# Blaizzy/mlx-audio-swift

Hardware: AMD Instinct MI355X
Metric: audio-seconds/sec (TTS gen+codec decode), Orpheus-3B batch 32 per GPU: value = whole-job aggregate over n_gpus, value_per_gpu = value / n_gpus (higher is better)
Workload: dtype bf16

## Files before the change

### include/mi_speech_debug.h

```cpp
#ifndef MI_SPEECH_DEBUG_H
#define MI_SPEECH_DEBUG_H
#include "mi_speech.h"
#ifdef __cplusplus
extern "C" {
#endif

mis_status mis_debug_launch_floor(int device, int n_kernels, int mode, int reps, double* us_per_kernel);
int32_t mis_debug_choose_split(int32_t items, int32_t k_tiles, int32_t waves_per_item, int32_t s_max);
mis_status mis_debug_occupy_cus(int device, int blocks, int threads, double seconds);
mis_status mis_debug_occupy_wait(void);
int32_t mis_debug_device_cus(int device);
int32_t mis_debug_sampler_failures(void);
int64_t mis_debug_whisper_weight_bytes(const mis_whisper* c);
mis_status mis_debug_mimi_decoder_tap(mis_mimi* m, const int32_t* codes, int batch, int n_q, int T, int stage, float* out, int64_t capacity,
                                      int32_t* channels, int64_t* length);

mis_status mis_debug_gemm_skinny(int device, const uint16_t* W, const uint16_t* W2, const uint16_t* X, const uint16_t* bias, int M, int N, int K,
                                 int epi, int R, int ksb, int U, int S, float* out, int64_t capacity, int32_t* report);
mis_status mis_debug_gemm_skinny_q(int device, int bits, int sb_dtype, const uint32_t* wq, const uint16_t* scales, const uint16_t* biases,
                                   const uint32_t* wq2, const uint16_t* scales2, const uint16_t* biases2, const uint16_t* X, const uint16_t* bias,
                                   int M, int N, int K, int epi, int R, int ksb, int S, float* out, int64_t capacity, int32_t* report);
mis_status mis_debug_gemm_pf(int device, const uint16_t* W, const uint16_t* W2, const uint16_t* X, const uint16_t* h, int M, int N, int K, int epi,
                             float* out, int64_t capacity, int32_t* report);

typedef struct mis_debug_attn_args {
    int32_t batch, Mpad, S, Nqkv, H, Hkv, D, Smax;
    int32_t cache_rows, append_only, first_schedule, cross, cross_len, out_ld, rope_in_dtype;
    int32_t qp_S, qp_KT;
    float scale, qk_eps, qp_eps;
    const float* qkv_part;
    const int32_t* pos;
    const uint8_t* active;
    const float *rope_cos, *rope_sin;
    const uint16_t *qnorm_w, *knorm_w;
    const uint16_t* qp_w;
// ... 92 lines not shown
```

### mlx-audio-swift_amd/_lib.py

```python
from __future__ import annotations

import ctypes as C
import os

_HERE = os.path.dirname(os.path.abspath(__file__))
LIB_PATH = os.environ.get("MIS_LIB_PATH") or os.path.join(_HERE, "libmi_speech.so")

MIS_OK = 0
STATUS_NAMES = {0: "ok", 1: "modelNotInitialized", 2: "generationFailed", 3: "invalidInput",
                4: "audioDecodingFailed", 5: "audioEncodingFailed", 6: "cancelled", 7: "device"}
MIS_F32, MIS_F16, MIS_BF16, MIS_I32 = 0, 1, 2, 3
EVENT_TOKEN, EVENT_INFO, EVENT_AUDIO = 0, 1, 2


class SnacConfigC(C.Structure):
    _fields_ = [("sampling_rate", C.c_int32), ("latent_dim", C.c_int32), ("decoder_dim", C.c_int32),
                ("n_decoder_rates", C.c_int32), ("decoder_rates", C.c_int32 * 8), ("codebook_size", C.c_int32),
                ("codebook_dim", C.c_int32), ("n_codebooks", C.c_int32), ("vq_strides", C.c_int32 * 8),
                ("noise", C.c_int32), ("depthwise", C.c_int32), ("attn_window_size", C.c_int32)]


class LmConfigC(C.Structure):
    _fields_ = [("hidden_size", C.c_int32), ("num_hidden_layers", C.c_int32), ("intermediate_size", C.c_int32),
                ("num_attention_heads", C.c_int32), ("num_key_value_heads", C.c_int32), ("head_dim", C.c_int32),
# ... 391 lines not shown
}

class AttnDebugArgsC(C.Structure):
    _fields_ = ([(n, C.c_int32) for n in ("batch", "Mpad", "S", "Nqkv", "H", "Hkv", "D", "Smax", "cache_rows", "append_only", "first_schedule",
                                          "cross", "cross_len", "out_ld", "rope_in_dtype", "qp_S", "qp_KT")] +
                [(n, C.c_float) for n in ("scale", "qk_eps", "qp_eps")] +
                [(n, _P) for n in ("qkv_part", "pos", "active", "rope_cos", "rope_sin", "qnorm_w", "knorm_w", "qp_w", "qp_bias", "qp_slabs",
                                   "qp_h_in", "qp_lnw", "qp_lnb", "kcache", "vtcache", "kcache_out", "vtcache_out", "out", "qp_h_out", "report")])


class CodecGemmDebugArgsC(C.Structure):
    _fields_ = ([(n, C.c_int32) for n in ("mode", "snake", "batch", "use_pack", "M", "K", "N", "Tin", "Tout", "s", "pad", "Cin", "ldx", "ldy",
                                          "x_lo", "dup_bias_n0", "split_k_ok", "taps", "dil", "noise_rng")] +
                [("noise_key", C.c_uint64), ("row_offset", C.c_int64)] +
                [(n, _P) for n in ("AT", "bias", "X", "R", "scale", "noise", "alpha", "ralpha", "row_ids", "Y", "report")])


DEBUG_SYMBOLS = {
    "mis_debug_launch_floor": (C.c_int, [C.c_int, C.c_int, C.c_int, C.c_int, C.POINTER(C.c_double)]),
    "mis_debug_occupy_cus": (C.c_int, [C.c_int, C.c_int, C.c_int, C.c_double]),
    "mis_debug_occupy_wait": (C.c_int, []),
    "mis_debug_device_cus": (C.c_int32, [C.c_int]),
    "mis_debug_sampler_failures": (C.c_int32, []),
    "mis_debug_choose_split": (C.c_int32, [C.c_int32, C.c_int32, C.c_int32, C.c_int32]),
    "mis_debug_gemm_skinny": (C.c_int, [C.c_int, _P, _P, _P, _P, C.c_int, C.c_int, C.c_int, C.c_int, C.c_int, C.c_int, C.c_int, C.c_int, _P,
                                        C.c_int64, _P]),
    "mis_debug_gemm_skinny_q": (C.c_int, [C.c_int, C.c_int, C.c_int, _P, _P, _P, _P, _P, _P, _P, _P, C.c_int, C.c_int, C.c_int, C.c_int, C.c_int,
                                          C.c_int, C.c_int, _P, C.c_int64, _P]),
    "mis_debug_gemm_pf": (C.c_int, [C.c_int, _P, _P, _P, _P, C.c_int, C.c_int, C.c_int, C.c_int, _P, C.c_int64, _P]),
    "mis_debug_attn_decode": (C.c_int, [C.c_int, C.POINTER(AttnDebugArgsC)]),
    "mis_debug_codec_gemm": (C.c_int, [C.c_int, C.POINTER(CodecGemmDebugArgsC)]),
    "mis_debug_codec_final": (C.c_int, [C.c_int, _P, _P, C.c_float, _P, _P, C.c_int, C.c_int, C.c_int, C.c_int, C.c_int, C.c_int, C.c_int64, _P]),
    "mis_debug_codec_hist": (C.c_int, [C.c_int, _P, _P, C.c_int, C.c_int, C.c_int, C.c_int, C.c_int, _P, _P]),
    "mis_debug_codec_embed": (C.c_int, [C.c_int, _P, C.c_int64, C.c_int64, C.c_int64, C.c_int64, _P, C.c_int, C.c_int, C.c_int, C.c_int, C.c_int,
                                        C.c_int, _P]),
    "mis_debug_codec_dw7": (C.c_int, [C.c_int, _P, _P, _P, C.c_int, C.c_int, C.c_int, C.c_int, _P]),
    "mis_debug_codec_vq_nearest": (C.c_int, [C.c_int, _P, _P, _P, C.c_int, C.c_int, C.c_int, C.c_int, _P]),
    "mis_debug_gemm_big": (C.c_int, [C.c_int, C.c_int, _P, _P, _P, _P, C.c_int, C.c_int, C.c_int, C.c_int, C.c_int, _P, _P]),
    "mis_debug_enc_layernorm": (C.c_int, [C.c_int, _P, _P, _P, C.c_int, C.c_int, C.c_float, _P, _P]),
    "mis_debug_enc_im2col3": (C.c_int, [C.c_int, _P, C.c_int, C.c_int, C.c_int, C.c_int, C.c_int, C.c_int, _P]),
    "mis_debug_enc_scatter_kv": (C.c_int, [C.c_int, _P, C.c_int, C.c_int, C.c_int, C.c_int, C.c_int, C.c_int, C.c_int, C.c_int, _P, _P]),
    "mis_debug_enc_attn_prefill": (C.c_int, [C.c_int, _P, C.c_int, _P, _P, C.c_int, C.c_int, C.c_int, C.c_int, C.c_int, C.c_int, _P, _P]),
    "mis_debug_whisper_embed_ln": (C.c_int, [C.c_int, _P, _P, _P, _P, _P, _P, _P, _P, C.c_int, C.c_int, C.c_int, C.c_int, C.c_int, _P, _P]),
    "mis_debug_whisper_suppress": (C.c_int, [C.c_int, _P, C.c_int, C.c_int, _P, C.c_int, _P, C.c_int, _P, _P, C.c_int]),
    "mis_debug_lm_embed_rmsnorm": (C.c_int, [C.c_int, _P, _P, _P, _P, _P, _P, C.c_int, C.c_int, C.c_float, C.c_int, C.c_int, _P, _P]),
    "mis_debug_lm_glue": (C.c_int, [C.c_int, _P, C.c_int, C.c_int, C.c_int, _P, _P, _P, C.c_float, _P, _P]),
# ... 55 lines not shown
```

### mlx-audio-swift_amd/csrc/lm_engine.hip

```cpp
#include <deque>
#include <map>
#include "common.h"
#include "kernels.h"
#include "lm_kernels.h"

#include <math.h>
#include <string.h>
#include <algorithm>
#include <chrono>
#include <functional>
#include <set>

#define ORPHEUS_END_OF_SPEECH 128258

struct mis_tts {
    int device = 0;
    hipStream_t stream = nullptr;
    mis_lm_config cfg{};
    mis_snac* codec = nullptr;
    int d = 0, L = 0, ff = 0, H = 0, Hkv = 0, D = 0, V = 0, Vpad = 0, Nqkv = 0;
    bool finalized = false, have_lm_head = false;
    std::set<std::string> loaded;

    DevBuf<bf16_t> emb;
// ... 16 lines not shown
    } q_qkv, q_o, q_gu, q_down, q_head;

    int batch = 0, Mpad = 0, Smax = 0;
    int S_qkv = 1, S_o = 1, S_down = 1;
    int r_part = 1;
    int r_gu = 2;
    int ksb_part = 4, ksb_gu = 4, ksb_head = 1;
    GemmArr a_qkv, a_o, a_down, a_head;
    GemmArr qa_gu, qa_head;
    DevBuf<bf16_t> kcache, vtcache;
    DevBuf<float> rope_cos, rope_sin;
    DevBuf<int32_t> ids, pos_cur, pos_next;
    DevBuf<uint8_t> active;
    DevBuf<bf16_t> h, x, attn_out, act, logits;
    DevBuf<float> qkv_part, part, e_buf, logits_f32, samp_l32;
    DevBuf<int32_t> prompt_mat, prompt_lens, step_counter, window, window_len, n_gen, tokens_out, all_ids, all_len,
        done_count, codes, n_codes, l0, l1, l2, row_map;
    DevBuf<float> pcm_tmp;
    DevBuf<bf16_t> pf_h, pf_x, pf_attn, pf_act, pf_xpk, pf_actpk;
    DevBuf<float> pf_qkv, pf_tmp;
    DevBuf<int32_t> pf_pos;
    DevBuf<uint8_t> pf_on;
    DevBuf<SamplerScratch> samp_scratch;
    hipGraphExec_t g_prefill = nullptr, g_decode = nullptr;
    bool shared_device = false;
    uint64_t graph_key = 0;
    bool use_graph = true;
    bool borrowed_stream = false;
    bool rope_csm = false;
    int profiling = 0;
    mis_tts_timing timing{};
    SamplerParams sp{};
};

static size_t layer_qkv_elems(const mis_tts* c) { return (size_t)c->Nqkv * c->d; }
static size_t layer_o_elems(const mis_tts* c) { return (size_t)c->d * c->H * c->D; }
static size_t layer_gu_elems(const mis_tts* c) { return (size_t)2 * c->ff * c->d; }
static size_t layer_down_elems(const mis_tts* c) { return (size_t)c->d * c->ff; }

extern "C" mis_status mis_tts_create(const mis_lm_config* cfg, mis_snac* codec, int device, mis_tts** out) {
    MIS_API_BEGIN
    MIS_REQUIRE(cfg && out, MIS_ERR_INVALID_INPUT, "null argument");
    MIS_REQUIRE(!codec || snac_device(codec) == device, MIS_ERR_INVALID_INPUT, "codec lives on another device");
    const int d = cfg->hidden_size, H = cfg->num_attention_heads, Hkv = cfg->num_key_value_heads;
    const int D = cfg->head_dim > 0 ? cfg->head_dim : (H > 0 ? d / H : 0);
    MIS_REQUIRE(d > 0 && cfg->num_hidden_layers > 0 && cfg->intermediate_size > 0 && H > 0 && Hkv > 0 && cfg->vocab_size > 0,
                MIS_ERR_INVALID_INPUT, "bad model dimensions");
// ... 14 lines not shown
    if (c->cfg.sample_rate <= 0) c->cfg.sample_rate = 24000;
    c->codec = codec;
    c->d = d; c->L = cfg->num_hidden_layers; c->ff = cfg->intermediate_size; c->H = H; c->Hkv = Hkv; c->D = D;
    c->V = cfg->vocab_size; c->Vpad = (int)round_up(c->V, 16); c->Nqkv = (H + 2 * Hkv) * D;
    c->emb.alloc((size_t)c->V * d);
    c->lm_head.alloc((size_t)c->Vpad * d);
    c->wqkv.alloc(layer_qkv_elems(c) * c->L);
    c->wo.alloc(layer_o_elems(c) * c->L);
    c->wgu.alloc(layer_gu_elems(c) * c->L);
    c->wdown.alloc(layer_down_elems(c) * c->L);
    c->norms.alloc((size_t)(2 * c->L + 1) * d);
    if (c->cfg.qk_norm) c->qknorm.alloc((size_t)2 * c->L * D);
    c->use_graph = getenv("MIS_NO_GRAPH") == nullptr;
    *out = c;
    MIS_API_END
}

extern "C" void mis_tts_destroy(mis_tts* c) {
    if (!c) return;
    (void)hipSetDevice(c->device);
    if (c->stream) (void)hipStreamSynchronize(c->stream);
    if (c->g_prefill) (void)hipGraphExecDestroy(c->g_prefill);
    if (c->g_decode) (void)hipGraphExecDestroy(c->g_decode);
    if (c->stream && !c->borrowed_stream) (void)hipStreamDestroy(c->stream);
    delete c;
}

static void place_matrix(mis_tts* c, const std::string& name, int64_t N, int64_t K) {
    hipStream_t s = c->stream;
    auto starts = [&](const char* p) { return name.rfind(p, 0) == 0; };
    if (name == "model.embed_tokens.weight") {
        MIS_REQUIRE(N == c->V && K == c->d, MIS_ERR_INVALID_INPUT, "embed_tokens shape mismatch");
        HIP_CHECK(hipMemcpyAsync(c->emb.p, c->staging.p, (size_t)N * K * 2, hipMemcpyDeviceToDevice, s));
        return;
    }
    if (name == "lm_head.weight") {
        MIS_REQUIRE(N == c->V && K == c->d, MIS_ERR_INVALID_INPUT, "lm_head shape mismatch");
        launch_pack_weight(c->staging.p, c->lm_head.p, c->V, c->d, c->Vpad / 16, 1, 0, s);
        c->have_lm_head = true;
        return;
    }
    MIS_REQUIRE(starts("model.layers."), MIS_ERR_INVALID_INPUT, "unexpected tensor %s", name.c_str());
    size_t p1 = strlen("model.layers.");
    size_t p2 = name.find('.', p1);
    MIS_REQUIRE(p2 != std::string::npos, MIS_ERR_INVALID_INPUT, "bad tensor name %s", name.c_str());
    int li = atoi(name.substr(p1, p2 - p1).c_str());
// ... 289 lines not shown
        decide(c->q_o, c->L, c->wo);
        decide(c->q_gu, 2 * c->L, c->wgu);
        decide(c->q_down, c->L, c->wdown);
        if (c->cfg.tie_word_embeddings) { c->q_head.on = false; c->q_head.q.release(); c->q_head.sb.release(); }
        else decide(c->q_head, 1, c->lm_head);
    }
    c->staging.release();
    c->raw_staging.release();
    c->finalized = true;
    MIS_API_END
}

static int env_int(const char* name, int dflt) {
    const char* v = getenv(name);
    return (v && *v) ? atoi(v) : dflt;
}
static int choose_split(int items, int KT, int ksb, const char* env, int s_max = 16) {
    return std::max(1, std::min(env_int(env, gemm_choose_split(items, KT, ksb, s_max)), 16));
}

static void destroy_graphs(mis_tts* c) {
    if (c->g_prefill) { (void)hipGraphExecDestroy(c->g_prefill); c->g_prefill = nullptr; }
    if (c->g_decode) { (void)hipGraphExecDestroy(c->g_decode); c->g_decode = nullptr; }
}

static void build_rope_tables(mis_tts* c) {
    const int D = c->D, half = D / 2;
    std::vector<float> inv(half);
    const float base = c->cfg.rope_theta, factor = c->cfg.rope_factor, low = c->cfg.rope_low_freq_factor,
                high = c->cfg.rope_high_freq_factor, old = c->cfg.rope_original_max_pos;
    for (int i = 0; i < half; ++i) {
        float expo = (float)(2 * i) / (float)D;
        float f = powf(base, expo);
        float wl = (float)(2.0f * (float)M_PI) * f;
        float low_wl = old / low, high_wl = old / high;
        float fs = (wl > low_wl) ? f * factor : f;
        bool med = (wl > high_wl) && (wl < low_wl);
        float smooth = (old / wl - low) / (high - low);
        float denom = (1.0f - smooth) / factor + smooth;
        float ff = med ? fs / denom : fs;
        if (c->cfg.rope_plain) ff = f;
        inv[i] = 1.0f / ff;
    }
    std::vector<float> cs((size_t)c->Smax * half), sn((size_t)c->Smax * half);
    if (c->rope_csm) marvis_rope_tables(D, base, factor, low, high, old, c->Smax, cs.data(), sn.data());
    else for (int p = 0; p < c->Smax; ++p)
// ... 717 lines not shown
        mix(ints, sizeof(ints));
        const void* hp[] = {hidden_mode ? (const void*)hm->hidden->p : nullptr, hidden_mode ? (const void*)hid_count.p : nullptr};
        mix(hp, sizeof(hp));
        if (key != c->graph_key) destroy_graphs(c);
        c->graph_key = key;
    }

    auto collect = [&](int prefill) {
        if (hidden_mode)
            hipLaunchKernelGGL(k_collect_hidden, dim3(batch), dim3(256), 0, s, c->x.p, c->active.p, hid_count.p, hm->hidden->p,
                               hid_rows, c->d, c->Mpad / 16, prefill);
    };
    auto prefill_body = [&]() {
        launch_prefill_feed(c->prompt_mat.p, c->prompt_lens.p, Lmax, c->step_counter.p, c->ids.p, c->active.p, batch, s);
        enqueue_layers(c);
        collect(1);
    };
    auto decode_body = [&]() {
        enqueue_lm_head(c);
        launch_sampler(c->sp, batch, s);
        enqueue_layers(c);
        collect(0);
    };
    auto capture = [&](hipGraphExec_t* exec, auto&& body) {
        hipGraph_t g = nullptr;
        HIP_CHECK(hipStreamBeginCapture(s, hipStreamCaptureModeThreadLocal));
        try { body(); } catch (...) { hipGraph_t dead = nullptr; (void)hipStreamEndCapture(s, &dead); if (dead) (void)hipGraphDestroy(dead); throw; }
        HIP_CHECK(hipStreamEndCapture(s, &g));
        HIP_CHECK(hipGraphInstantiate(exec, g, nullptr, nullptr, 0));
        HIP_CHECK(hipGraphDestroy(g));
    };

    hipEvent_t ev[4];
    for (auto& e : ev) HIP_CHECK(hipEventCreate(&e));
    auto t_host0 = std::chrono::steady_clock::now();
    HIP_CHECK(hipEventRecord(ev[0], s));
    if (prefill_batched_ok(c, Lmax)) {
        prefill_batched(c, c->prompt_mat.p, c->prompt_lens.p, lens, Lmax);
        collect(1);
    } else {
        if (c->use_graph && !c->g_prefill) capture(&c->g_prefill, prefill_body);
        for (int j = 0; j < Lmax; ++j) {
            if (c->use_graph) HIP_CHECK(hipGraphLaunch(c->g_prefill, s)); else prefill_body();
        }
    }
    HIP_CHECK(hipEventRecord(ev[1], s));
    {
        std::vector<uint8_t> ones(batch, 1);
        HIP_CHECK(hipMemcpyAsync(c->active.p, ones.data(), batch, hipMemcpyHostToDevice, s));
        HIP_CHECK(hipStreamSynchronize(s));
    }
    if (c->use_graph && !c->g_decode) capture(&c->g_decode, decode_body);
    int steps = 0;
    const int poll = cb ? 8 : 32;
    std::vector<int32_t> host_ngen(batch, 0), host_tok;
    bool cancelled = false;
    PinnedBuf<int32_t> done_pin(1);
    PinnedBuf<unsigned> fail_pin(batch);
    int32_t* done_host = done_pin.p;
    *done_host = 0;
    while (steps < max_tokens) {
        int chunk = std::min(poll, max_tokens - steps);
        for (int i = 0; i < chunk; ++i) {
            if (c->use_graph) HIP_CHECK(hipGraphLaunch(c->g_decode, s)); else decode_body();
        }
        steps += chunk;
        HIP_CHECK(hipMemcpyAsync(done_host, c->done_count.p, 4, hipMemcpyDeviceToHost, s));
        sampler_fail_flags_async(c->samp_scratch.p, batch, fail_pin.p, s);
        if (cb) {
            host_tok.resize((size_t)batch * max_tokens);
            HIP_CHECK(hipMemcpyAsync(host_ngen.data(), c->n_gen.p, batch * 4, hipMemcpyDeviceToHost, s));
            HIP_CHECK(hipMemcpyAsync(host_tok.data(), c->tokens_out.p, host_tok.size() * 4, hipMemcpyDeviceToHost, s));
        }
        HIP_CHECK(hipStreamSynchronize(s));
        if (sampler_fail_flags_any(fail_pin.p, batch)) {
            sampler_note_failure(c->samp_scratch.p, batch, s);
            for (auto& e : ev) (void)hipEventDestroy(e);
            throw SamplerTimeout{};
        }
        if (cb) {
            for (int b = 0; b < batch; ++b)
                for (; emitted[b] < host_ngen[b]; ++emitted[b]) {
                    int32_t t = host_tok[(size_t)b * max_tokens + emitted[b]];
                    if (hidden_mode && t == hm->stop_id) continue;
                    cb(user, b, MIS_EVENT_TOKEN, &t, 1);
                }
        }
// ... 582 lines not shown
```

### mlx-audio-swift_amd/csrc/lm_kernels.h

```cpp
#pragma once
#include "common.h"

__host__ __device__ __forceinline__ size_t xpk_index(int m, int k, int MT) {
    return ((((size_t)(k >> 5) * MT + (m >> 4)) * 64) + (((k & 31) >> 3) << 4) + (m & 15)) * 8 + (k & 7);
}

enum { EPI_PARTIAL = 0, EPI_BF16 = 1, EPI_SILU_MUL = 2, EPI_GELU_PACKED = 3, EPI_SILU_PACKED = 4 };

void launch_convert_to_bf16(const void* src, int dtype, bf16_t* dst, size_t n, hipStream_t s);
void launch_bf16_to_f32(const bf16_t* src, float* dst, size_t n, hipStream_t s);
void launch_dequant_affine(const uint32_t* wq, const void* scales, const void* biases, int sb_dtype, bf16_t* dst, int N, int K,
                           int group, int bits, hipStream_t s);
void launch_pack_weight(const bf16_t* src, bf16_t* dst, int N, int K, int NT, int tile_stride, int tile_offset,
                        hipStream_t s);
void launch_synth_fill_bf16(bf16_t* dst, size_t n, uint64_t key, float amp, int plus_one, hipStream_t s);

void launch_prefill_feed(const int32_t* prompt, const int32_t* lens, int Lmax, int* step_counter, int32_t* ids,
                         uint8_t* active, int batch, hipStream_t s);
void launch_embed_rmsnorm(const bf16_t* emb, const int32_t* ids, const uint8_t* active, int* pos_cur, int* pos_next,
                          const bf16_t* wnorm, bf16_t* h, bf16_t* x, int d, int vocab, float eps, int batch, int Mpad,
                          hipStream_t s);
void launch_reduce_residual_rmsnorm(const float* slabs, int S, int Mpad, int N, bf16_t* h, const bf16_t* wnorm,
                                    bf16_t* x, float eps, hipStream_t s, const bf16_t* ln_bias = nullptr);
void launch_gemm_skinny(int epi, int R, int ksb, const bf16_t* Wp, const bf16_t* X, void* out, int NT, int KT, int S,
// ... 97 lines not shown
    int32_t* n_gen;
    int32_t* tokens_out;
    int tokens_stride;
    int32_t* all_ids;
    int32_t* all_len;
    int all_stride;
    int32_t* next_ids;
    uint8_t* active;
    int32_t* done_count;
    int32_t* step_override;
    float temperature, top_p, penalty;
    int penalty_flavor;
    uint64_t seed;
    int64_t row_offset;
    int frame_constrained;
    int audio_offset;
    int lo, hi;
    int eos_id;
    int max_tokens;
    unsigned long long* dbg;
    int path_resolved;
    int force_multi;
    int spin;
};
void sampler_resolve(SamplerParams& p, bool multi_launch_only);
void sampler_fail_flags_async(SamplerScratch* scratch, int batch, unsigned* host_flags, hipStream_t s);
bool sampler_fail_flags_any(const unsigned* host_flags, int batch);
void sampler_note_failure(SamplerScratch* scratch, int batch, hipStream_t s);
void launch_sampler(const SamplerParams& p, int batch, hipStream_t s, bool multi_launch_only = false);
```

### mlx-audio-swift_amd/csrc/lm_sampler.hip

```cpp
#include "common.h"
#include "lm_kernels.h"
#include "sampler_math.h"
#include <vector>
#include <atomic>
#include <mutex>

#define SAMP_NT 256
#define ORPHEUS_AUDIO_OFFSET 128266

typedef unsigned long long u64;
static_assert(SAMP_MAX_CHUNKS <= 64, "per-chunk quantities are reduced one per lane");


__device__ __forceinline__ void allowed_range(const SamplerParams& p, int step, int& lo, int& hi) {
    const int V = p.vocab;
    lo = p.lo;
    hi = (p.hi <= 0 || p.hi > V) ? V : p.hi;
    if (p.frame_constrained) {
        lo = (p.audio_offset > 0 ? p.audio_offset : ORPHEUS_AUDIO_OFFSET) + (step % 7) * 4096;
        hi = lo + 4096;
        if (hi > V) hi = V;
        if (lo > hi) lo = hi;
    }
    if (lo < 0) lo = 0;
// ... 515 lines not shown
#define SC_WALL(k) do { if (p.dbg && blockIdx.y == 0 && threadIdx.x == 0) p.dbg[16 + 4 * blockIdx.x + (k)] = wall_clock64(); } while (0)
static_assert(SC_NB == SAMP_CLUSTER_NB, "exchange slots per row (lm_kernels.h)");
__device__ __forceinline__ u64 sc_load(const u64* p) { return __hip_atomic_load(p, __ATOMIC_RELAXED, __HIP_MEMORY_SCOPE_AGENT); }
__device__ __forceinline__ void sc_store(u64* p, u64 v) { __hip_atomic_store(p, v, __ATOMIC_RELAXED, __HIP_MEMORY_SCOPE_AGENT); }
__device__ __forceinline__ unsigned sc_key32(float f) { const unsigned u = __float_as_uint(f); return (u & 0x80000000u) ? ~u : (u | 0x80000000u); }
__device__ __forceinline__ float sc_unkey32(unsigned k) { return __uint_as_float((k & 0x80000000u) ? (k & 0x7fffffffu) : ~k); }
__device__ __forceinline__ bool sc_row_barrier(unsigned int* sync, unsigned target, int spin_limit, unsigned long long* dbg = nullptr) {
    __shared__ int ok;
    asm volatile("s_waitcnt vmcnt(0)" ::: "memory");
    __syncthreads();
    if (dbg && blockIdx.x == 0 && blockIdx.y == 0 && threadIdx.x == 0) *dbg = __builtin_readcyclecounter();
    if (threadIdx.x == 0) {
        __hip_atomic_fetch_add(sync, 1u, __ATOMIC_RELAXED, __HIP_MEMORY_SCOPE_AGENT);
        int good = 0;
        for (int it = 0; it < spin_limit; ++it) {
            if ((int)(__hip_atomic_load(sync, __ATOMIC_RELAXED, __HIP_MEMORY_SCOPE_AGENT) - target) >= 0) { good = 1; break; }
            __builtin_amdgcn_s_sleep(1);
        }
        ok = good;
    }
    __syncthreads();
    return ok != 0;
}
__global__ void __launch_bounds__(SC_NT) k_samp_cluster(SamplerParams p, int spin_limit) {
    __shared__ u64 hist[256];
    __shared__ u64 sh[SC_NT / 64];
    __shared__ u64 redk[SC_NT / 64];
    __shared__ u64 kept[SC_NB];
    __shared__ __attribute__((aligned(16))) uint32_t stage[SC_NT * SC_PER / 2];
    __shared__ int pen_id[64];
    __shared__ float pen_val[64];
    __shared__ int swin[64];
    __shared__ int n_pen;
    __shared__ unsigned s_bin;
    __shared__ u64 s_below;
    __shared__ int s_token;
    const int c = blockIdx.x, b = blockIdx.y, tid = threadIdx.x;
    SC_STAMP(0);
    SC_WALL(0);
    if (row_skipped(p, b)) return;
    SamplerScratch* sc = p.scratch + b;
    const int step = row_step(p, b);
    int lo, hi;
    allowed_range(p, step, lo, hi);
    bf16_t* logits = p.logits + (size_t)b * p.Vpad;
    const int my0 = (c * SC_NT + tid) * SC_PER;
    const bool penalise = p.penalty > 0.0f && p.penalty != 1.0f && p.window;
    const int32_t* wl_src = penalise ? p.window_len + b : reinterpret_cast<const int32_t*>(&sc->c_sync);
    const int32_t* win_src = penalise ? p.window + (size_t)b * p.ctx + (tid < p.ctx ? tid : 0) : reinterpret_cast<const int32_t*>(&sc->c_sync);
    const int wl_raw = *wl_src;
    const int win_raw = *win_src;
    const unsigned sync_now = __hip_atomic_load(&sc->c_sync, __ATOMIC_RELAXED, __HIP_MEMORY_SCOPE_AGENT);
    if (__hip_atomic_load(&sc->c_fail, __ATOMIC_RELAXED, __HIP_MEMORY_SCOPE_AGENT) != 0u) spin_limit = 0;
    const int wlen_all = penalise ? wl_raw : 0;
    typedef unsigned int u32x4_t __attribute__((ext_vector_type(4)));
    u32x4_t q[3];
    {
        const u32x4_t* lp = reinterpret_cast<const u32x4_t*>(logits);
        const int n16 = p.Vpad >> 3;
        const int c0 = c * (SC_NT * SC_PER / 8);
#pragma unroll
        for (int j = 0; j < 3; ++j) {
            const int ch = c0 + tid + j * SC_NT;
            q[j] = lp[ch < n16 ? ch : n16 - 1];
        }
    }
    const int wl = min(wlen_all, 64);
    if (penalise && tid < p.ctx && tid >= p.ctx - wlen_all && tid - (p.ctx - wlen_all) < 64) swin[tid - (p.ctx - wlen_all)] = win_raw;
    unsigned base = 0;
// ... 9 lines not shown
    __syncthreads();
    base = (unsigned)redk[0];
    if (penalise) {
        const float pen = bf16_round_f32(p.penalty);
        if (tid < wl) {
            const int id = swin[tid];
            bool first = id >= 0 && id < p.vocab && id / (SC_NT * SC_PER) == c;
            for (int j = 0; j < tid; ++j) first = first && (swin[j] != id);
            if (first) {
                const float l = bf16_to_f32(logits[id]);
                const bf16_t v = f32_to_bf16((l < 0.0f) ? l * pen : __fdiv_rn(l, pen));
                logits[id] = v;
                const int slot = atomicAdd(&n_pen, 1);
                pen_id[slot] = id; pen_val[slot] = bf16_to_f32(v);
            }
        }
    }
    float l[SC_PER];
    {
#pragma unroll
        for (int j = 0; j < 3; ++j)
            if (tid + j * SC_NT < SC_NT * SC_PER / 8) reinterpret_cast<u32x4_t*>(stage)[tid + j * SC_NT] = q[j];
        __syncthreads();
#pragma unroll
        for (int j = 0; j < SC_PER / 4; ++j) {
            const uint2 w = *reinterpret_cast<const uint2*>(stage + tid * (SC_PER / 2) + 2 * j);
            l[4 * j] = bf16_to_f32((bf16_t)(w.x & 0xffffu)); l[4 * j + 1] = bf16_to_f32((bf16_t)(w.x >> 16));
            l[4 * j + 2] = bf16_to_f32((bf16_t)(w.y & 0xffffu)); l[4 * j + 3] = bf16_to_f32((bf16_t)(w.y >> 16));
        }
    }
    __syncthreads();
    {
        const int np = n_pen;
        for (int k = 0; k < np; ++k) {
            const int d = pen_id[k] - my0;
            const float v = pen_val[k];
#pragma unroll
            for (int j = 0; j < SC_PER; ++j) l[j] = (d == j) ? v : l[j];
        }
    }
    SC_STAMP(1);
    SC_WALL(1);
    u64 bestk = 0;
#pragma unroll
    for (int j = 0; j < SC_PER; ++j) {
        const int i = my0 + j;
        const u64 k = ((u64)sc_key32(l[j]) << 32) | (unsigned)(~(unsigned)i);
        bestk = (i >= lo && i < hi && k > bestk) ? k : bestk;
    }
    if (p.temperature == 0.0f) {
#pragma unroll
        for (int o = 32; o > 0; o >>= 1) {
            const unsigned lo32 = __shfl_xor((unsigned)bestk, o, 64), hi32 = __shfl_xor((unsigned)(bestk >> 32), o, 64);
            const u64 ok = ((u64)hi32 << 32) | lo32;
            bestk = ok > bestk ? ok : bestk;
        }
    } else {
        bestk = (u64)wave_max_u32((unsigned)(bestk >> 32)) << 32;
    }
    if ((tid & 63) == 0) redk[tid >> 6] = bestk;
    __syncthreads();
    if (tid == 0) {
        u64 m = 0;
#pragma unroll
        for (int w = 0; w < SC_NT / 64; ++w) m = redk[w] > m ? redk[w] : m;
        sc_store(&sc->x_max[c], m);
    }
    SC_STAMP(2);
    SC_WALL(2);
    bool alive = sc_row_barrier(&sc->c_sync, base + 1u * SC_NB, spin_limit, p.dbg ? p.dbg + 12 : nullptr);
    SC_STAMP(3);
    SC_WALL(3);
    u64 rowk = 0;
#pragma unroll
    for (int k = 0; k < SC_NB; ++k) { const u64 v = sc_load(&sc->x_max[k]); rowk = v > rowk ? v : rowk; }
    const float best = rowk ? sc_unkey32((unsigned)(rowk >> 32)) : -INFINITY;
    const int best_i = rowk ? (int)~(unsigned)rowk : 0x7fffffff;
    u64 Zk = 0;
    bool mine_blk = false;
    if (p.temperature == 0.0f || !alive) {
        if (tid == 0) __hip_atomic_fetch_add(&sc->c_sync, (unsigned)(SC_ARRIVALS - 1), __ATOMIC_RELAXED, __HIP_MEMORY_SCOPE_AGENT);
        if (tid == 0 && alive && best_i != 0x7fffffff) s_token = best_i;
        mine_blk = c == 0;
        Zk = 1;
    } else {
        const float xmax = __fdiv_rn(best, p.temperature);
        float e[SC_PER];
#pragma unroll
        for (int j = 0; j < SC_PER; ++j) {
            const int i = my0 + j;
            const float x = __fdiv_rn(l[j], p.temperature);
            const float y = fminf(x - xmax, 0.0f);
            e[j] = (i >= lo && i < hi) ? det_exp_dev(y) : 0.0f;
            if ((j & 3) == 3) __builtin_amdgcn_sched_barrier(0);
        }
        SC_STAMP(4);
#pragma unroll
        for (int j = 0; j < SC_PER; ++j) {
            const u64 E = (u64)(e[j] * E_SCALE);
            if (E) atomicAdd(&hist[__float_as_uint(e[j]) >> 24], E);
        }
        __syncthreads();
        SC_STAMP(5);
        if (tid < 256) sc_store(&sc->x_hist1[c][tid], hist[tid]);
        alive = sc_row_barrier(&sc->c_sync, base + 2u * SC_NB, spin_limit, p.dbg ? p.dbg + 13 : nullptr) && alive;
        SC_STAMP(6);
        u64 mine = 0;
#pragma unroll
        for (int k = 0; k < SC_NB; ++k) mine += tid < 256 ? sc_load(&sc->x_hist1[k][tid]) : 0;
        unsigned kstar = 0;
        const bool nucleus = p.top_p > 0.0f && p.top_p < 1.0f;
        if (nucleus) {
            u64 Z = 0;
// ... 47 lines not shown
                const int w = tid >> 6, ln = tid & 63;
                const u64 v = wave_sum_u64((table[w * 256 + ln] + table[w * 256 + 64 + ln]) + (table[w * 256 + 128 + ln] + table[w * 256 + 192 + ln]));
                if (ln == 0) kept[w] = v + sc_load(&sc->x_above[w]);
            }
        } else {
            if (tid == 0) __hip_atomic_fetch_add(&sc->c_sync, 1u, __ATOMIC_RELAXED, __HIP_MEMORY_SCOPE_AGENT);
            u64* table = reinterpret_cast<u64*>(stage);
            if (tid < 256) {
#pragma unroll
                for (int k = 0; k < SC_NB; ++k) table[k * 256 + tid] = sc_load(&sc->x_hist1[k][tid]);
            }
            __syncthreads();
            if (tid < SC_NB * 64) {
                const int w = tid >> 6, ln = tid & 63;
                const u64 v = wave_sum_u64((table[w * 256 + ln] + table[w * 256 + 64 + ln]) + (table[w * 256 + 128 + ln] + table[w * 256 + 192 + ln]));
                if (ln == 0) kept[w] = v;
            }
        }
        __syncthreads();
        SC_STAMP(10);
        u64 before = 0;
#pragma unroll
        for (int k = 0; k < SC_NB; ++k) { const u64 v = kept[k]; Zk += v; before += (k < c) ? v : 0; }
        mine = 0;
#pragma unroll
        for (int j = 0; j < SC_PER; ++j) mine += ((__float_as_uint(e[j]) >> 16) >= kstar) ? (u64)(e[j] * E_SCALE) : 0;
        u64 Zblk = 0;
        const u64 incl = block_scan_incl_1024(mine, sh, &Zblk);
        const u64 row = (u64)(p.row_offset + b);
        const u64 a = p.seed ^ (0xD1B54A32D192ED03ull * (row + 1));
        const u64 rnd = mis_splitmix64(mis_splitmix64(a) + (u64)step);
        const u64 r = __umul64hi(rnd, Zk);
        const u64 excl = before + incl - mine;
        bool hit = false;
        if (mine > 0 && r >= excl && r < excl + mine) {
            u64 run = excl;
#pragma unroll
            for (int j = 0; j < SC_PER; ++j) {
                const u64 Ek = ((__float_as_uint(e[j]) >> 16) >= kstar) ? (u64)(e[j] * E_SCALE) : 0;
                run += Ek;
                if (!hit && Ek && run > r) { s_token = my0 + j; hit = true; }
            }
        }
        mine_blk = r >= before && r < before + Zblk;
        SC_STAMP(11);
    }
    if (!alive) {
        if (tid == 0) __hip_atomic_store(&sc->c_fail, 1u, __ATOMIC_RELAXED, __HIP_MEMORY_SCOPE_AGENT);
        if (c != 0) return;
    } else if (Zk ? !mine_blk : c != 0) return;
    __syncthreads();
    if (tid == 0) {
        const int token = s_token;
        if (p.tokens_out && step < p.tokens_stride) p.tokens_out[(size_t)b * p.tokens_stride + step] = token;
        if (p.n_gen && !p.step_override) p.n_gen[b] = step + 1;
        if (p.window && p.ctx > 0) {
            int32_t* win = p.window + (size_t)b * p.ctx;
            int wl = p.window_len[b];
            if (wl < p.ctx) { wl++; p.window_len[b] = wl; }
            for (int j = p.ctx - wl; j < p.ctx - 1; ++j) win[j] = win[j + 1];
            win[p.ctx - 1] = token;
        }
        if (p.next_ids) p.next_ids[b] = token;
        if (token == p.eos_id) {
            if (p.active) p.active[b] = 0;
            if (p.done_count) atomicAdd(p.done_count, 1);
        } else {
// ... 15 lines not shown
void sampler_fail_flags_async(SamplerScratch* scratch, int batch, unsigned* host_flags, hipStream_t s) {
    HIP_CHECK(hipMemcpy2DAsync(host_flags, sizeof(unsigned), &scratch[0].c_fail, sizeof(SamplerScratch), sizeof(unsigned), (size_t)batch,
                               hipMemcpyDeviceToHost, s));
}
bool sampler_fail_flags_any(const unsigned* host_flags, int batch) {
    bool any = false;
    for (int b = 0; b < batch; ++b) any = any || host_flags[b] != 0;
    return any;
}
void sampler_note_failure(SamplerScratch* scratch, int batch, hipStream_t s) {
    g_sampler_failures.fetch_add(1);
    sampler_scratch_init(scratch, batch, s);
    HIP_CHECK(hipStreamSynchronize(s));
}
bool sampler_check_failed(SamplerScratch* scratch, int batch, hipStream_t s) {
    if (!scratch || batch <= 0) return false;
    std::vector<unsigned> f(batch, 0u);
    sampler_fail_flags_async(scratch, batch, f.data(), s);
    HIP_CHECK(hipStreamSynchronize(s));
    const bool any = sampler_fail_flags_any(f.data(), batch);
    if (any) sampler_note_failure(scratch, batch, s);
    return any;
}
static bool sampler_cluster_fits(int batch) {
    static std::mutex mu;
    static std::map<int, int> capacity;
    int dev = 0;
    if (hipGetDevice(&dev) != hipSuccess) return false;
    std::lock_guard<std::mutex> lk(mu);
    auto it = capacity.find(dev);
    if (it == capacity.end()) {
        int per_cu = 0, cap = 0;
        hipDeviceProp_t prop{};
        if (hipGetDeviceProperties(&prop, dev) == hipSuccess &&
            hipOccupancyMaxActiveBlocksPerMultiprocessor(&per_cu, k_samp_cluster, SC_NT, 0) == hipSuccess)
            cap = std::min(per_cu, 2) * prop.multiProcessorCount;
        it = capacity.emplace(dev, cap).first;
    }
    return SC_NB * batch <= it->second;
}

void sampler_resolve(SamplerParams& p, bool multi_launch_only) {
    const char* ew = getenv("MIS_SAMPLER_WIDE");
    const char* es = getenv("MIS_SAMPLER_SPIN");
    p.path_resolved = 1;
    p.force_multi = (multi_launch_only || (ew && atoi(ew) != 0)) ? 1 : 0;
    p.spin = es ? (atoi(es) > 0 ? atoi(es) : 0) : (1 << 22);
}

void sampler_plan(int vocab, int* n_chunks, int* chunk_w) {
    int nc = (vocab + 4095) / 4096;
    if (nc > SAMP_MAX_CHUNKS) nc = SAMP_MAX_CHUNKS;
    if (nc < 1) nc = 1;
    int cw = (vocab + nc - 1) / nc;
    cw = (cw + 7) / 8 * 8;
    *n_chunks = (vocab + cw - 1) / cw;
    *chunk_w = cw;
}

void launch_sampler(const SamplerParams& p_in, int batch, hipStream_t s, bool multi_launch_only) {
    MIS_REQUIRE(p_in.scratch && p_in.n_chunks >= 1 && p_in.n_chunks <= SAMP_MAX_CHUNKS && p_in.chunk_w > 0, MIS_ERR_GENERATION_FAILED,
                "sampler scratch not configured");
    SamplerParams p = p_in;
    if (!p.path_resolved) sampler_resolve(p, multi_launch_only);
    const bool multi = multi_launch_only || p.force_multi != 0;
    {
        const int hi = (p.hi <= 0 || p.hi > p.vocab) ? p.vocab : p.hi, lo = p.lo < 0 ? 0 : p.lo;
        const bool narrow = p.frame_constrained == 1 || (!p.frame_constrained && hi - lo <= SN_W);
        if (narrow && !multi && !p.logits32 && p.penalty_flavor == 0) {
            hipLaunchKernelGGL(k_samp_narrow, dim3(batch), dim3(SN_NT), 0, s, p);
            return;
        }
    }
    if (!multi && !p.logits32 && p.penalty_flavor == 0 && p.vocab <= SC_NB * SC_NT * SC_PER && p.Vpad % 16 == 0 && p.ctx <= 64 &&
        sampler_cluster_fits(batch)) {
        hipLaunchKernelGGL(k_samp_cluster, dim3(SC_NB, batch), dim3(SC_NT), 0, s, p, p.spin);
        return;
    }
    dim3 g2(p.n_chunks, batch);
    hipLaunchKernelGGL(k_samp_prepare, dim3(batch), dim3(64), 0, s, p);
    hipLaunchKernelGGL(k_samp_max, g2, dim3(SAMP_NT), 0, s, p);
    if (p.temperature == 0.0f) {
        hipLaunchKernelGGL(k_samp_pick, dim3(batch), dim3(SAMP_NT), 0, s, p, 1);
        return;
    }
    hipLaunchKernelGGL(k_samp_exp, g2, dim3(SAMP_NT), 0, s, p);
    int nucleus = (p.top_p > 0.0f && p.top_p < 1.0f) ? 1 : 0;
    if (nucleus) hipLaunchKernelGGL(k_samp_hist2, g2, dim3(SAMP_NT), 0, s, p);
    hipLaunchKernelGGL(k_samp_mass, g2, dim3(SAMP_NT), 0, s, p, nucleus);
    hipLaunchKernelGGL(k_samp_pick, dim3(batch), dim3(SAMP_NT), 0, s, p, 0);
}
```

Measured before the change: 185.1.

## Stride cluster sampler element ownership and skip decoder layers on final step

The cluster sampler now defaults to a strided element-to-thread mapping for the staged logits read. The inverse-CDF pick transposes the kept probabilities back to contiguous order through shared memory, but only in the block that owns the draw. This is meant to avoid shared-memory bank conflicts in the per-thread strided reads. Separately, the last decode step launches a new graph that runs only the LM head and sampler, skipping the transformer layers whose KV writes are never used; it adds an extra captured graph and an environment opt-out.

New measurement: 185.2, median of 2. Within noise of the previous version (+0.1%).

```diff
diff --git a/include/mi_speech_debug.h b/include/mi_speech_debug.h
--- a/include/mi_speech_debug.h
+++ b/include/mi_speech_debug.h
@@ -11,6 +11,8 @@
 mis_status mis_debug_occupy_wait(void);
 int32_t mis_debug_device_cus(int device);
 int32_t mis_debug_sampler_failures(void);
+int32_t mis_debug_sampler_last_path(void);
+int32_t mis_debug_sampler_cluster_rows(int device);
 int64_t mis_debug_whisper_weight_bytes(const mis_whisper* c);
 mis_status mis_debug_mimi_decoder_tap(mis_mimi* m, const int32_t* codes, int batch, int n_q, int T, int stage, float* out, int64_t capacity,
                                       int32_t* channels, int64_t* length);
diff --git a/mlx-audio-swift_amd/_lib.py b/mlx-audio-swift_amd/_lib.py
--- a/mlx-audio-swift_amd/_lib.py
+++ b/mlx-audio-swift_amd/_lib.py
@@ -437,6 +437,8 @@
     "mis_debug_occupy_wait": (C.c_int, []),
     "mis_debug_device_cus": (C.c_int32, [C.c_int]),
     "mis_debug_sampler_failures": (C.c_int32, []),
+    "mis_debug_sampler_last_path": (C.c_int32, []),
+    "mis_debug_sampler_cluster_rows": (C.c_int32, [C.c_int]),
     "mis_debug_choose_split": (C.c_int32, [C.c_int32, C.c_int32, C.c_int32, C.c_int32]),
     "mis_debug_gemm_skinny": (C.c_int, [C.c_int, _P, _P, _P, _P, C.c_int, C.c_int, C.c_int, C.c_int, C.c_int, C.c_int, C.c_int, C.c_int, _P,
                                         C.c_int64, _P]),
diff --git a/mlx-audio-swift_amd/csrc/lm_engine.hip b/mlx-audio-swift_amd/csrc/lm_engine.hip
--- a/mlx-audio-swift_amd/csrc/lm_engine.hip
+++ b/mlx-audio-swift_amd/csrc/lm_engine.hip
@@ -62,7 +62,7 @@
     DevBuf<int32_t> pf_pos;
     DevBuf<uint8_t> pf_on;
     DevBuf<SamplerScratch> samp_scratch;
-    hipGraphExec_t g_prefill = nullptr, g_decode = nullptr;
+    hipGraphExec_t g_prefill = nullptr, g_decode = nullptr, g_final = nullptr;
     bool shared_device = false;
     uint64_t graph_key = 0;
     bool use_graph = true;
@@ -123,6 +123,7 @@
     if (c->stream) (void)hipStreamSynchronize(c->stream);
     if (c->g_prefill) (void)hipGraphExecDestroy(c->g_prefill);
     if (c->g_decode) (void)hipGraphExecDestroy(c->g_decode);
+    if (c->g_final) (void)hipGraphExecDestroy(c->g_final);
     if (c->stream && !c->borrowed_stream) (void)hipStreamDestroy(c->stream);
     delete c;
 }
@@ -458,6 +459,7 @@
 static void destroy_graphs(mis_tts* c) {
     if (c->g_prefill) { (void)hipGraphExecDestroy(c->g_prefill); c->g_prefill = nullptr; }
     if (c->g_decode) { (void)hipGraphExecDestroy(c->g_decode); c->g_decode = nullptr; }
+    if (c->g_final) { (void)hipGraphExecDestroy(c->g_final); c->g_final = nullptr; }
 }
 
 static void build_rope_tables(mis_tts* c) {
@@ -1221,6 +1223,11 @@
         enqueue_layers(c);
         collect(0);
     };
+    const bool short_last = !hidden_mode && !(getenv("MIS_FULL_LAST_STEP") && atoi(getenv("MIS_FULL_LAST_STEP")) != 0);
+    auto final_body = [&]() {
+        enqueue_lm_head(c);
+        launch_sampler(c->sp, batch, s);
+    };
     auto capture = [&](hipGraphExec_t* exec, auto&& body) {
         hipGraph_t g = nullptr;
         HIP_CHECK(hipStreamBeginCapture(s, hipStreamCaptureModeThreadLocal));
@@ -1250,6 +1257,7 @@
         HIP_CHECK(hipStreamSynchronize(s));
     }
     if (c->use_graph && !c->g_decode) capture(&c->g_decode, decode_body);
+    if (c->use_graph && short_last && !c->g_final) capture(&c->g_final, final_body);
     int steps = 0;
     const int poll = cb ? 8 : 32;
     std::vector<int32_t> host_ngen(batch, 0), host_tok;
@@ -1261,7 +1269,11 @@
     while (steps < max_tokens) {
         int chunk = std::min(poll, max_tokens - steps);
         for (int i = 0; i < chunk; ++i) {
-            if (c->use_graph) HIP_CHECK(hipGraphLaunch(c->g_decode, s)); else decode_body();
+            if (short_last && steps + i + 1 == max_tokens) {
+                if (c->use_graph) HIP_CHECK(hipGraphLaunch(c->g_final, s)); else final_body();
+            } else {
+                if (c->use_graph) HIP_CHECK(hipGraphLaunch(c->g_decode, s)); else decode_body();
+            }
         }
         steps += chunk;
         HIP_CHECK(hipMemcpyAsync(done_host, c->done_count.p, 4, hipMemcpyDeviceToHost, s));
diff --git a/mlx-audio-swift_amd/csrc/lm_kernels.h b/mlx-audio-swift_amd/csrc/lm_kernels.h
--- a/mlx-audio-swift_amd/csrc/lm_kernels.h
+++ b/mlx-audio-swift_amd/csrc/lm_kernels.h
@@ -143,6 +143,7 @@
     int path_resolved;
     int force_multi;
     int spin;
+    int consecutive;
 };
 void sampler_resolve(SamplerParams& p, bool multi_launch_only);
 void sampler_fail_flags_async(SamplerScratch* scratch, int batch, unsigned* host_flags, hipStream_t s);
diff --git a/mlx-audio-swift_amd/csrc/lm_sampler.hip b/mlx-audio-swift_amd/csrc/lm_sampler.hip
--- a/mlx-audio-swift_amd/csrc/lm_sampler.hip
+++ b/mlx-audio-swift_amd/csrc/lm_sampler.hip
@@ -561,6 +561,7 @@
     __syncthreads();
     return ok != 0;
 }
+template <int STRIDED>
 __global__ void __launch_bounds__(SC_NT) k_samp_cluster(SamplerParams p, int spin_limit) {
     __shared__ u64 hist[256];
     __shared__ u64 sh[SC_NT / 64];
@@ -583,7 +584,9 @@
     int lo, hi;
     allowed_range(p, step, lo, hi);
     bf16_t* logits = p.logits + (size_t)b * p.Vpad;
-    const int my0 = (c * SC_NT + tid) * SC_PER;
+    const int blk0 = c * SC_NT * SC_PER;
+    const int my0 = blk0 + tid * SC_PER;
+    auto id_of = [&](int j) { return STRIDED ? blk0 + j * SC_NT + tid : my0 + j; };
     const bool penalise = p.penalty > 0.0f && p.penalty != 1.0f && p.window;
     const int32_t* wl_src = penalise ? p.window_len + b : reinterpret_cast<const int32_t*>(&sc->c_sync);
     const int32_t* win_src = penalise ? p.window + (size_t)b * p.ctx + (tid < p.ctx ? tid : 0) : reinterpret_cast<const int32_t*>(&sc->c_sync);
@@ -639,8 +642,13 @@
         for (int j = 0; j < 3; ++j)
             if (tid + j * SC_NT < SC_NT * SC_PER / 8) reinterpret_cast<u32x4_t*>(stage)[tid + j * SC_NT] = q[j];
         __syncthreads();
-#pragma unroll
-        for (int j = 0; j < SC_PER / 4; ++j) {
+        if (STRIDED) {
+            const bf16_t* sb = reinterpret_cast<const bf16_t*>(stage);
+#pragma unroll
+            for (int j = 0; j < SC_PER; ++j) l[j] = bf16_to_f32(sb[j * SC_NT + tid]);
+        }
+#pragma unroll
+        for (int j = 0; j < (STRIDED ? 0 : SC_PER / 4); ++j) {
             const uint2 w = *reinterpret_cast<const uint2*>(stage + tid * (SC_PER / 2) + 2 * j);
             l[4 * j] = bf16_to_f32((bf16_t)(w.x & 0xffffu)); l[4 * j + 1] = bf16_to_f32((bf16_t)(w.x >> 16));
             l[4 * j + 2] = bf16_to_f32((bf16_t)(w.y & 0xffffu)); l[4 * j + 3] = bf16_to_f32((bf16_t)(w.y >> 16));
@@ -650,10 +658,10 @@
     {
         const int np = n_pen;
         for (int k = 0; k < np; ++k) {
-            const int d = pen_id[k] - my0;
+            const int d = pen_id[k] - id_of(0);
             const float v = pen_val[k];
 #pragma unroll
-            for (int j = 0; j < SC_PER; ++j) l[j] = (d == j) ? v : l[j];
+            for (int j = 0; j < SC_PER; ++j) l[j] = (d == (STRIDED ? j * SC_NT : j)) ? v : l[j];
         }
     }
     SC_STAMP(1);
@@ -661,7 +669,7 @@
     u64 bestk = 0;
 #pragma unroll
     for (int j = 0; j < SC_PER; ++j) {
-        const int i = my0 + j;
+        const int i = id_of(j);
         const u64 k = ((u64)sc_key32(l[j]) << 32) | (unsigned)(~(unsigned)i);
         bestk = (i >= lo && i < hi && k > bestk) ? k : bestk;
     }
@@ -705,7 +713,7 @@
         float e[SC_PER];
 #pragma unroll
         for (int j = 0; j < SC_PER; ++j) {
-            const int i = my0 + j;
+            const int i = id_of(j);
             const float x = __fdiv_rn(l[j], p.temperature);
             const float y = fminf(x - xmax, 0.0f);
             e[j] = (i >= lo && i < hi) ? det_exp_dev(y) : 0.0f;
@@ -799,27 +807,69 @@
         u64 before = 0;
 #pragma unroll
         for (int k = 0; k < SC_NB; ++k) { const u64 v = kept[k]; Zk += v; before += (k < c) ? v : 0; }
-        mine = 0;
-#pragma unroll
-        for (int j = 0; j < SC_PER; ++j) mine += ((__float_as_uint(e[j]) >> 16) >= kstar) ? (u64)(e[j] * E_SCALE) : 0;
-        u64 Zblk = 0;
-        const u64 incl = block_scan_incl_1024(mine, sh, &Zblk);
         const u64 row = (u64)(p.row_offset + b);
         const u64 a = p.seed ^ (0xD1B54A32D192ED03ull * (row + 1));
         const u64 rnd = mis_splitmix64(mis_splitmix64(a) + (u64)step);
         const u64 r = __umul64hi(rnd, Zk);
-        const u64 excl = before + incl - mine;
-        bool hit = false;
-        if (mine > 0 && r >= excl && r < excl + mine) {
-            u64 run = excl;
-#pragma unroll
-            for (int j = 0; j < SC_PER; ++j) {
-                const u64 Ek = ((__float_as_uint(e[j]) >> 16) >= kstar) ? (u64)(e[j] * E_SCALE) : 0;
-                run += Ek;
-                if (!hit && Ek && run > r) { s_token = my0 + j; hit = true; }
-            }
-        }
-        mine_blk = r >= before && r < before + Zblk;
+        if (STRIDED) {
+            mine_blk = r >= before && r < before + kept[c];
+            if (mine_blk) {
+                float* tf = reinterpret_cast<float*>(stage);
+                float ec[SC_PER];
+#pragma unroll
+                for (int qr = 0; qr < 2; ++qr) {
+                    if (qr) __syncthreads();
+#pragma unroll
+                    for (int k = 0; k < SC_PER / 2; ++k) {
+                        const float v = e[qr * (SC_PER / 2) + k];
+                        tf[k * SC_NT + tid] = ((__float_as_uint(v) >> 16) >= kstar) ? v : 0.0f;
+                    }
+                    __syncthreads();
+                    if ((tid >> 9) == qr) {
+                        const u32x4_t* src = reinterpret_cast<const u32x4_t*>(tf) + (tid & 511) * (SC_PER / 4);
+#pragma unroll
+                        for (int k = 0; k < SC_PER / 4; ++k) {
+                            const u32x4_t w = src[k];
+                            ec[4 * k] = __uint_as_float(w.x); ec[4 * k + 1] = __uint_as_float(w.y);
+                            ec[4 * k + 2] = __uint_as_float(w.z); ec[4 * k + 3] = __uint_as_float(w.w);
+                        }
+                    }
+                }
+                mine = 0;
+#pragma unroll
+                for (int j = 0; j < SC_PER; ++j) mine += (u64)(ec[j] * E_SCALE);
+                const u64 incl = block_scan_incl_1024(mine, sh, nullptr);
+                const u64 excl = before + incl - mine;
+                bool hit = false;
+                if (mine > 0 && r >= excl && r < excl + mine) {
+                    u64 run = excl;
+#pragma unroll
+                    for (int j = 0; j < SC_PER; ++j) {
+                        const u64 Ek = (u64)(ec[j] * E_SCALE);
+                        run += Ek;
+                        if (!hit && Ek && run > r) { s_token = my0 + j; hit = true; }
+                    }
+                }
+            }
+        } else {
+            mine = 0;
+#pragma unroll
+            for (int j = 0; j < SC_PER; ++j) mine += ((__float_as_uint(e[j]) >> 16) >= kstar) ? (u64)(e[j] * E_SCALE) : 0;
+            u64 Zblk = 0;
+            const u64 incl = block_scan_incl_1024(mine, sh, &Zblk);
+            const u64 excl = before + incl - mine;
+            bool hit = false;
+            if (mine > 0 && r >= excl && r < excl + mine) {
+                u64 run = excl;
+#pragma unroll
+                for (int j = 0; j < SC_PER; ++j) {
+                    const u64 Ek = ((__float_as_uint(e[j]) >> 16) >= kstar) ? (u64)(e[j] * E_SCALE) : 0;
+                    run += Ek;
+                    if (!hit && Ek && run > r) { s_token = my0 + j; hit = true; }
+                }
+            }
+            mine_blk = r >= before && r < before + Zblk;
+        }
         SC_STAMP(11);
     }
     if (!alive) {
@@ -881,28 +931,41 @@
     if (any) sampler_note_failure(scratch, batch, s);
     return any;
 }
-static bool sampler_cluster_fits(int batch) {
+static int sampler_cluster_capacity() {
     static std::mutex mu;
     static std::map<int, int> capacity;
     int dev = 0;
-    if (hipGetDevice(&dev) != hipSuccess) return false;
+    if (hipGetDevice(&dev) != hipSuccess) return 0;
     std::lock_guard<std::mutex> lk(mu);
     auto it = capacity.find(dev);
     if (it == capacity.end()) {
-        int per_cu = 0, cap = 0;
+        int per_cu = 0, per_cu0 = 0, cap = 0;
         hipDeviceProp_t prop{};
         if (hipGetDeviceProperties(&prop, dev) == hipSuccess &&
-            hipOccupancyMaxActiveBlocksPerMultiprocessor(&per_cu, k_samp_cluster, SC_NT, 0) == hipSuccess)
-            cap = std::min(per_cu, 2) * prop.multiProcessorCount;
+            hipOccupancyMaxActiveBlocksPerMultiprocessor(&per_cu, k_samp_cluster<1>, SC_NT, 0) == hipSuccess &&
+            hipOccupancyMaxActiveBlocksPerMultiprocessor(&per_cu0, k_samp_cluster<0>, SC_NT, 0) == hipSuccess)
+            cap = std::min(std::min(per_cu, per_cu0), 2) * prop.multiProcessorCount;
         it = capacity.emplace(dev, cap).first;
     }
-    return SC_NB * batch <= it->second;
+    return it->second;
+}
+static bool sampler_cluster_fits(int batch) { return SC_NB * batch <= sampler_cluster_capacity(); }
+static std::atomic<int> g_sampler_last_path{0};
+extern "C" int32_t mis_debug_sampler_last_path(void) { return g_sampler_last_path.load(); }
+extern "C" int32_t mis_debug_sampler_cluster_rows(int device) {
+    int prev = 0;
+    if (hipGetDevice(&prev) != hipSuccess || hipSetDevice(device) != hipSuccess) return 0;
+    const int rows = sampler_cluster_capacity() / SC_NB;
+    (void)hipSetDevice(prev);
+    return rows;
 }
 
 void sampler_resolve(SamplerParams& p, bool multi_launch_only) {
     const char* ew = getenv("MIS_SAMPLER_WIDE");
     const char* es = getenv("MIS_SAMPLER_SPIN");
+    const char* ec = getenv("MIS_SAMPLER_CONSECUTIVE");
     p.path_resolved = 1;
+    p.consecutive = (ec && atoi(ec) != 0) ? 1 : 0;
     p.force_multi = (multi_launch_only || (ew && atoi(ew) != 0)) ? 1 : 0;
     p.spin = es ? (atoi(es) > 0 ? atoi(es) : 0) : (1 << 22);
 }
@@ -928,14 +991,18 @@
         const bool narrow = p.frame_constrained == 1 || (!p.frame_constrained && hi - lo <= SN_W);
         if (narrow && !multi && !p.logits32 && p.penalty_flavor == 0) {
             hipLaunchKernelGGL(k_samp_narrow, dim3(batch), dim3(SN_NT), 0, s, p);
+            g_sampler_last_path.store(1);
             return;
         }
     }
     if (!multi && !p.logits32 && p.penalty_flavor == 0 && p.vocab <= SC_NB * SC_NT * SC_PER && p.Vpad % 16 == 0 && p.ctx <= 64 &&
         sampler_cluster_fits(batch)) {
-        hipLaunchKernelGGL(k_samp_cluster, dim3(SC_NB, batch), dim3(SC_NT), 0, s, p, p.spin);
+        if (p.consecutive) hipLaunchKernelGGL(k_samp_cluster<0>, dim3(SC_NB, batch), dim3(SC_NT), 0, s, p, p.spin);
+        else hipLaunchKernelGGL(k_samp_cluster<1>, dim3(SC_NB, batch), dim3(SC_NT), 0, s, p, p.spin);
+        g_sampler_last_path.store(p.consecutive ? 3 : 2);
         return;
     }
+    g_sampler_last_path.store(4);
     dim3 g2(p.n_chunks, batch);
     hipLaunchKernelGGL(k_samp_prepare, dim3(batch), dim3(64), 0, s, p);
     hipLaunchKernelGGL(k_samp_max, g2, dim3(SAMP_NT), 0, s, p);
```
